# RainbowZL0/swin-unet-image-fusion

Measured on AMD Instinct MI355X. Metric: fused image-pairs/sec at 256x256, win=8, higher is better.
Workload: dtype bf16; 1 GPU; B=16/GPU 256x256 IR/visible pairs, win=8, 5-level Swin-UNet fusion forward (BASELINE configs[1]); global_batch=16, precision_mode=fast, residual_stream=fp32, hip_graph=True, steps_in_flight=3, kernel_schedule=throughput, collective=none, weights=random-init (numpy PCG64 recipe, seed 0)

## Files before the change

### swin_unet_image_fusion_amd/csrc/kernels_patchrr.hip

```cpp
#include "kernels_patchrr.h"

#include <algorithm>

#include "win_frag.h"

namespace swf {
namespace {

using namespace wf;

struct PrrArgs {
    const float* in[2]; float* out[2]; const float* skip[2]; const char* packed[2];
    int B, H, W, Cin;
    int mh, mw, Hm, Wm;
    int Ho, Wo;
    int K, N, Cout, M;
};

template <int KS, int NT>
struct PRR {
    static constexpr int NFRAG = NT * KS * 2;
    static constexpr int NV = NT * 16;
    static constexpr size_t p_vec = size_t(NFRAG) * 1024;
    static constexpr size_t p_total = p_vec + size_t(3) * 2 * NV * 4;
};

template <int KS, int NT, int DEC, int CIN1, int TPW>
__global__ __launch_bounds__(256) void patch_rr_kernel(PrrArgs a) {
    using P = PRR<KS, NT>;
    constexpr int NV = P::NV;
    __shared__ float lvec[3 * 2 * NV];
    const int s = blockIdx.y, tid = threadIdx.x, lane = tid & 63, wave = tid >> 6;
    const int r = lane & 31, hf = lane >> 5;
    fill_vectors<3 * NV / 4, 256>(lvec, a.packed[s] + P::p_vec, a.packed[s] + P::p_vec + (3 * NV / 4) * 16, tid);
    const __amdgpu_buffer_rsrc_t wrs = __builtin_amdgcn_make_buffer_rsrc(const_cast<char*>(a.packed[s]), 0, (int)P::p_total, 0x00020000);
    const unsigned loff = (unsigned)lane * 16u;
    auto WA = [&](int nt, int ks, int hl) {
        return __builtin_bit_cast(u32x4, __builtin_amdgcn_raw_buffer_load_b128(wrs, loff, ((nt * KS + ks) * 2 + hl) * 1024, 0));
    };
    __syncthreads();
    const float* vbias = lvec + hf * NV;
    const float* vgam = lvec + 2 * NV + hf * NV;
    const float* vbet = lvec + 4 * NV + hf * NV;
    const float* in = a.in[s];
    const int K = a.K, N = a.N, Cin = a.Cin;
    const float invN = 1.0f / (float)N;
    const f32x16 zero16 = {0.f, 0.f, 0.f, 0.f, 0.f, 0.f, 0.f, 0.f, 0.f, 0.f, 0.f, 0.f, 0.f, 0.f, 0.f, 0.f};

    const int ngroup = (a.M + 32 * TPW - 1) / (32 * TPW);
    for (int grp = blockIdx.x * 4 + wave; grp < ngroup; grp += gridDim.x * 4) {
        int tok[TPW], base[TPW][4];
        bool live[TPW];
#pragma unroll
        for (int u = 0; u < TPW; ++u) {
            const int t = (grp * TPW + u) * 32 + r;
            live[u] = t < a.M;
            const int tc = live[u] ? t : a.M - 1;
            tok[u] = tc;
            if constexpr (DEC) {
                const int mx = tc % a.Wm, t2 = tc / a.Wm, my = t2 % a.Hm, b = t2 / a.Hm;
                base[u][0] = ((b * a.H + my) * a.W + mx) * Cin;
                base[u][1] = base[u][2] = base[u][3] = 0;
            } else {
                const int ox = tc % a.Wo, t2 = tc / a.Wo, oy = t2 % a.Ho, b = t2 / a.Ho;
                const int my = reflect_br(oy, a.Hm), mx = reflect_br(ox, a.Wm);
                const int iy0 = reflect_br(2 * my, a.H), iy1 = reflect_br(2 * my + 1, a.H);
                const int ix0 = reflect_br(2 * mx, a.W), ix1 = reflect_br(2 * mx + 1, a.W);
                base[u][0] = ((b * a.H + iy0) * a.W + ix0) * Cin;
                base[u][1] = ((b * a.H + iy0) * a.W + ix1) * Cin;
                base[u][2] = ((b * a.H + iy1) * a.W + ix0) * Cin;
                base[u][3] = ((b * a.H + iy1) * a.W + ix1) * Cin;
            }
        }
        f32x16 acc[TPW][NT];
#pragma unroll
        for (int u = 0; u < TPW; ++u)
#pragma unroll
            for (int nt = 0; nt < NT; ++nt) acc[u][nt] = zero16;
        float xin[TPW][KS][8];
        {
            int pqk = 0, ck = 8 * hf;
            if constexpr (!DEC && !CIN1) {
                while (ck >= Cin) { ck -= Cin; ++pqk; }
            }
#pragma unroll
            for (int ks = 0; ks < KS; ++ks) {
#pragma unroll
                for (int u = 0; u < TPW; ++u) {
#pragma unroll
                    for (int j = 0; j < 8; ++j) xin[u][ks][j] = 0.f;
                    if constexpr (CIN1) {
                        if (hf == 0) {
                            xin[u][ks][0] = in[base[u][0]]; xin[u][ks][1] = in[base[u][1]];
                            xin[u][ks][2] = in[base[u][2]]; xin[u][ks][3] = in[base[u][3]];
                        }
                    } else {
                        const int k0 = 16 * ks + 8 * hf;
                        if (k0 < K) {
                            int off;
                            if constexpr (DEC) off = base[u][0] + k0;
                            else off = (pqk == 0 ? base[u][0] : pqk == 1 ? base[u][1] : pqk == 2 ? base[u][2] : base[u][3]) + ck;
                            const float4 x0 = *reinterpret_cast<const float4*>(in + off), x1 = *reinterpret_cast<const float4*>(in + off + 4);
                            xin[u][ks][0] = x0.x; xin[u][ks][1] = x0.y; xin[u][ks][2] = x0.z; xin[u][ks][3] = x0.w;
                            xin[u][ks][4] = x1.x; xin[u][ks][5] = x1.y; xin[u][ks][6] = x1.z; xin[u][ks][7] = x1.w;
                        }
                    }
                }
                if constexpr (!DEC && !CIN1) {
                    ck += 16;
                    while (ck >= Cin) { ck -= Cin; ++pqk; }
                }
            }
        }
        constexpr bool DEC_VEC = DEC != 0;
        constexpr bool SKIP_EARLY = DEC_VEC && NT <= 3;
        int oidx[DEC_VEC ? TPW : 1][DEC_VEC ? NT : 1][4];
        float4 skv[DEC_VEC ? TPW : 1][DEC_VEC ? NT : 1][4];
        auto dec_offsets = [&](int u) {
            const int t = tok[u];
            const int mx = t % a.Wm, t2 = t / a.Wm, my = t2 % a.Hm, b = t2 / a.Hm;
            int pq = 0, c = 4 * hf;
            while (c >= a.Cout) { c -= a.Cout; ++pq; }
#pragma unroll
            for (int nt = 0; nt < NT; ++nt)
#pragma unroll
                for (int g = 0; g < 4; ++g) {
                    const int yy = my * 2 + (pq >> 1), xx = mx * 2 + (pq & 1);
                    const bool ok = live[u] && 32 * nt + 8 * g + 4 * hf < N && yy < a.Ho && xx < a.Wo;
                    oidx[u][nt][g] = ok ? ((b * a.Ho + yy) * a.Wo + xx) * a.Cout + c : -1;
                    c += 8;
                    while (c >= a.Cout) { c -= a.Cout; ++pq; }
                }
        };
        auto load_skips = [&](int u) {
#pragma unroll
            for (int nt = 0; nt < NT; ++nt)
#pragma unroll
                for (int g = 0; g < 4; ++g)
                    skv[u][nt][g] = (a.skip[s] && oidx[u][nt][g] >= 0) ? *reinterpret_cast<const float4*>(a.skip[s] + oidx[u][nt][g])
                                                                       : make_float4(0.f, 0.f, 0.f, 0.f);
        };
        if constexpr (DEC_VEC) {
            if (a.Cout > 1) {
#pragma unroll
                for (int u = 0; u < TPW; ++u) {
                    dec_offsets(u);
                    if constexpr (SKIP_EARLY) load_skips(u);
                }
            }
        }
        u32x4 wr[2][NT][2];
        SWF_WF_FENCE();
#pragma unroll
        for (int nt = 0; nt < NT; ++nt) { wr[0][nt][0] = WA(nt, 0, 0); wr[0][nt][1] = WA(nt, 0, 1); }
#pragma unroll
        for (int ks = 0; ks < KS; ++ks) {
            if (ks + 1 < KS) {
#pragma unroll
                for (int nt = 0; nt < NT; ++nt) { wr[(ks + 1) & 1][nt][0] = WA(nt, ks + 1, 0); wr[(ks + 1) & 1][nt][1] = WA(nt, ks + 1, 1); }
            }
            SWF_WF_FENCE();
            u32x4 bh[TPW], bl[TPW];
#pragma unroll
            for (int u = 0; u < TPW; ++u) split8(xin[u][ks], bh[u], bl[u]);
#pragma unroll
            for (int nt = 0; nt < NT; ++nt)
#pragma unroll
                for (int u = 0; u < TPW; ++u) acc[u][nt] = mma3(wr[ks & 1][nt][0], wr[ks & 1][nt][1], bh[u], bl[u], acc[u][nt]);
        }
#pragma unroll
        for (int u = 0; u < TPW; ++u) {
            float sum = 0.f;
#pragma unroll
            for (int nt = 0; nt < NT; ++nt)
#pragma unroll
                for (int i = 0; i < 16; ++i) {
                    acc[u][nt][i] += vbias[nt * 16 + i];
                    sum += acc[u][nt][i];
                }
            const float mean = sum_halves(sum) * invN;
            float q = 0.f;
#pragma unroll
            for (int nt = 0; nt < NT; ++nt)
#pragma unroll
                for (int i = 0; i < 16; ++i) {
                    const float d = acc[u][nt][i] - mean;
                    q += (32 * nt + rho(i, hf) < N) ? d * d : 0.f;
                }
            const float rstd = __builtin_amdgcn_rsqf(sum_halves(q) * invN + 1e-5f);
            const int t = tok[u];
            if constexpr (DEC_VEC) {
                if (a.Cout > 1) {
                    if constexpr (!SKIP_EARLY) load_skips(u);
                }
            }
#pragma unroll
            for (int nt = 0; nt < NT; ++nt)
#pragma unroll
                for (int g = 0; g < 4; ++g) {
                    const int n0 = 32 * nt + 8 * g + 4 * hf;
                    if (n0 < N) {
                        float y[4];
#pragma unroll
                        for (int j = 0; j < 4; ++j) {
                            const int i = 4 * g + j;
                            const float z = (acc[u][nt][i] - mean) * rstd * vgam[nt * 16 + i] + vbet[nt * 16 + i];
                            y[j] = z > 0.f ? z : __builtin_amdgcn_exp2f(z * kLog2e) - 1.0f;
                        }
                        if constexpr (!DEC) {
                            if (live[u]) *reinterpret_cast<float4*>(a.out[s] + (int64_t)t * N + n0) = make_float4(y[0], y[1], y[2], y[3]);
                        } else if (a.Cout == 1) {
                            if (live[u]) {
                                const int mx = t % a.Wm, t2 = t / a.Wm, my = t2 % a.Hm, b = t2 / a.Hm;
#pragma unroll
                                for (int j = 0; j < 4; ++j) {
                                    const int yy = my * 2 + (j >> 1), xx = mx * 2 + (j & 1);
                                    if (yy < a.Ho && xx < a.Wo) {
                                        const int64_t o = ((int64_t)b * a.Ho + yy) * a.Wo + xx;
                                        a.out[s][o] = a.skip[s] ? y[j] + a.skip[s][o] : y[j];
                                    }
                                }
                            }
                        } else {
                            const int o = oidx[u][nt][g];
                            if (o >= 0) {
                                const float4 k4 = skv[u][nt][g];
                                *reinterpret_cast<float4*>(a.out[s] + o) = make_float4(y[0] + k4.x, y[1] + k4.y, y[2] + k4.z, y[3] + k4.w);
                            }
                        }
                    }
                }
        }
    }
}

struct PrrPackArgs { const float* w; const float* bias; const float* gamma; const float* beta; char* dst; int K, N; };

template <int KS, int NT>
__global__ __launch_bounds__(256) void patch_rr_pack_kernel(PrrPackArgs a) {
    using P = PRR<KS, NT>;
    const int gtid = blockIdx.x * blockDim.x + threadIdx.x, gsz = gridDim.x * blockDim.x;
    for (int idx = gtid; idx < P::NFRAG * 512; idx += gsz) {
        const int f = idx >> 9, lane = (idx >> 3) & 63, e = idx & 7, r = lane & 31, hf = lane >> 5;
        const int hl = f & 1, ks = (f >> 1) % KS, nt = f / (2 * KS);
        const int n = 32 * nt + r, k = 16 * ks + 8 * hf + e;
        const float val = (n < a.N && k < a.K) ? a.w[(int64_t)n * a.K + k] : 0.f;
        const bf16 hi = (bf16)val;
        reinterpret_cast<bf16*>(a.dst)[idx] = hl ? (bf16)(val - (float)hi) : hi;
    }
    float* vec = reinterpret_cast<float*>(a.dst + P::p_vec);
    for (int i = gtid; i < 3 * 2 * P::NV; i += gsz) {
        const int which = i / (2 * P::NV), hf = (i / P::NV) & 1, j = i % P::NV, nt = j >> 4, reg = j & 15;
        const int n = 32 * nt + rho(reg, hf);
        const float* src = which == 0 ? a.bias : which == 1 ? a.gamma : a.beta;
        vec[i] = (n < a.N && src) ? src[n] : 0.f;
    }
}

bool shape_class(int decoder, int Cin, int Cout, int mh, int mw, int* ks, int* nt) {
    if (mh != 2 || mw != 2 || Cin <= 0 || Cout <= 0) return false;
    const int K = decoder ? Cin : 4 * Cin, N = decoder ? 4 * Cout : Cout;
    if (decoder) {
        if (Cin % 8 || !(Cout == 1 || Cout % 4 == 0)) return false;
    } else {
        if (!(Cin == 1 || Cin % 8 == 0) || Cout % 4) return false;
    }
    *ks = (K + 15) / 16;
    *nt = (N + 31) / 32;
    const int k = *ks, n = *nt;
    if (decoder) return (k == 2 && n == 1) || (k == 3 && n == 3) || (k == 6 && n == 6);
    return (k == 1 && n == 1 && Cin == 1) || (k == 6 && n == 2) || (k == 12 && n == 3);
}

template <int KS, int NT, int DEC, int CIN1, int TPW>
int launch_t(const PrrArgs& a, int nstream, hipStream_t stream) {
    const int ngroup = (a.M + 32 * TPW - 1) / (32 * TPW);
    const int gx = std::max(1, std::min((ngroup + 3) / 4, 8 * num_cus() / nstream));
    hipLaunchKernelGGL((patch_rr_kernel<KS, NT, DEC, CIN1, TPW>), dim3(gx, nstream), dim3(256), 0, stream, a);
    return check_launch("patch_rr");
}

}

bool patch_rr_supported(int decoder, int Cin, int Cout, int mh, int mw) {
    int ks, nt;
    return shape_class(decoder, Cin, Cout, mh, mw, &ks, &nt);
}

size_t patch_rr_packed_bytes(int decoder, int Cin, int Cout, int mh, int mw) {
    int ks, nt;
    if (!shape_class(decoder, Cin, Cout, mh, mw, &ks, &nt)) return 0;
    return align_up(size_t(nt) * ks * 2 * 1024 + size_t(3) * 2 * nt * 16 * 4, 256);
}

int pack_patch_rr(int decoder, int Cin, int Cout, int mh, int mw, const float* weight, const float* bias, const float* gamma,
                  const float* beta, void* dst, hipStream_t stream) {
    int ks, nt;
    if (!shape_class(decoder, Cin, Cout, mh, mw, &ks, &nt)) return fail(SWF_ERR_UNSUPPORTED, "pack_patch_rr: shape not covered");
    PrrPackArgs a{weight, bias, gamma, beta, static_cast<char*>(dst), decoder ? Cin : 4 * Cin, decoder ? 4 * Cout : Cout};
#define SWF_PRR_PACK(KS_, NT_) if (ks == KS_ && nt == NT_) { hipLaunchKernelGGL((patch_rr_pack_kernel<KS_, NT_>), dim3(32), dim3(256), 0, stream, a); return check_launch("pack_patch_rr"); }
    SWF_PRR_PACK(1, 1) SWF_PRR_PACK(2, 1) SWF_PRR_PACK(3, 3) SWF_PRR_PACK(6, 2) SWF_PRR_PACK(6, 6) SWF_PRR_PACK(12, 3)
#undef SWF_PRR_PACK
    return fail(SWF_ERR_UNSUPPORTED, "pack_patch_rr: shape class");
}

int launch_patch_rr(const PatchFusedDesc& d, const void* const* packed, int nstream, hipStream_t stream) {
    int ks, nt;
    if (!shape_class(d.decoder, d.Cin, d.Cout, d.mh, d.mw, &ks, &nt)) return fail(SWF_ERR_UNSUPPORTED, "patch_rr: shape not covered");
    if (d.M <= 0 || d.M > INT32_MAX - 64) return fail(SWF_ERR_UNSUPPORTED, "patch_rr: token count");
    const int64_t in_elems = (int64_t)d.B * d.H * d.W * d.Cin;
    const int64_t out_elems = d.decoder ? (int64_t)d.B * d.Ho * d.Wo * d.Cout : d.M * (int64_t)d.N;
    if (in_elems >= (int64_t(1) << 31) || out_elems >= (int64_t(1) << 31)) return fail(SWF_ERR_UNSUPPORTED, "patch_rr: tensor too large");
    PrrArgs a{};
    uintptr_t bits = 0;
    for (int s = 0; s < nstream; ++s) {
        if (!packed || !packed[s]) return fail(SWF_ERR_NULL, "patch_rr: packed image missing");
        a.in[s] = d.in[s]; a.out[s] = d.out[s]; a.skip[s] = d.skip[s]; a.packed[s] = static_cast<const char*>(packed[s]);
        bits |= reinterpret_cast<uintptr_t>(d.in[s]) | reinterpret_cast<uintptr_t>(d.out[s]) | reinterpret_cast<uintptr_t>(d.skip[s]) |
                reinterpret_cast<uintptr_t>(packed[s]);
    }
    if (bits % 16) return fail(SWF_ERR_UNSUPPORTED, "patch_rr: tensors must be 16-byte aligned");
    a.B = d.B; a.H = d.H; a.W = d.W; a.Cin = d.Cin; a.mh = d.mh; a.mw = d.mw; a.Hm = d.Hm; a.Wm = d.Wm; a.Ho = d.Ho; a.Wo = d.Wo;
    a.K = d.K; a.N = d.N; a.Cout = d.Cout; a.M = (int)d.M;
    if (!d.decoder) {
        if (ks == 1 && nt == 1 && d.Cin == 1) return launch_t<1, 1, 0, 1, 2>(a, nstream, stream);
        if (ks == 6 && nt == 2) return launch_t<6, 2, 0, 0, 2>(a, nstream, stream);
        if (ks == 12 && nt == 3) return launch_t<12, 3, 0, 0, 1>(a, nstream, stream);
    } else {
        if (ks == 2 && nt == 1) return launch_t<2, 1, 1, 0, 2>(a, nstream, stream);
        if (ks == 3 && nt == 3) return launch_t<3, 3, 1, 0, 1>(a, nstream, stream);
        if (ks == 6 && nt == 6) return launch_t<6, 6, 1, 0, 1>(a, nstream, stream);
    }
    return fail(SWF_ERR_UNSUPPORTED, "patch_rr: no instantiation for k-steps %d, tiles %d (decoder %d)", ks, nt, d.decoder);
}

}
```

Before: 8971 pairs/s.

## Add software-pipelined patch-merge kernel with LDS-staged weights and input prefetch

Adds a pipelined variant of the fused patch-merge/expand kernel. It stages the packed weight and vector image into LDS once per block, then prefetches the next token group's inputs (and decoder skip values) while the current group's MMAs and LayerNorm/ELU epilogue run. By default it is used for two encoder shapes, the Cin=1 stem and the ks12/nt3 merge, each with its own blocks-per-CU grid setting. An env var can turn it off or route every shape through it. The cost is higher register pressure from the double-buffered inputs and dynamic LDS use, which can lower occupancy.

```diff
diff --git a/swin_unet_image_fusion_amd/csrc/kernels_patchrr.hip b/swin_unet_image_fusion_amd/csrc/kernels_patchrr.hip
--- a/swin_unet_image_fusion_amd/csrc/kernels_patchrr.hip
+++ b/swin_unet_image_fusion_amd/csrc/kernels_patchrr.hip
@@ -234,6 +234,270 @@
     }
 }
 
+template <int KS, int NT, int DEC, int CIN1, int TPW, int PF>
+__global__ __launch_bounds__(256) void patch_rr_pipe_kernel(PrrArgs a) {
+    using P = PRR<KS, NT>;
+    constexpr int NV = P::NV;
+    constexpr int TOTAL16 = (int)(P::p_total / 16), PER = (TOTAL16 + 255) / 256;
+    extern __shared__ __attribute__((aligned(16))) char prr_smem[];
+    const int s = blockIdx.y, tid = threadIdx.x, lane = tid & 63, wave = tid >> 6;
+    const int r = lane & 31, hf = lane >> 5;
+    const u32x4* lw = reinterpret_cast<const u32x4*>(prr_smem) + lane;
+    const float* lvec = reinterpret_cast<const float*>(prr_smem + P::p_vec);
+    const float* vbias = lvec + hf * NV;
+    const float* vgam = lvec + 2 * NV + hf * NV;
+    const float* vbet = lvec + 4 * NV + hf * NV;
+    const float* in = a.in[s];
+    const int K = a.K, N = a.N, Cin = a.Cin;
+    const float invN = 1.0f / (float)N;
+    const f32x16 zero16 = {0.f, 0.f, 0.f, 0.f, 0.f, 0.f, 0.f, 0.f, 0.f, 0.f, 0.f, 0.f, 0.f, 0.f, 0.f, 0.f};
+    constexpr bool DEC_VEC = DEC != 0;
+    const bool pair_in = CIN1 && !(a.W & 1) && 2 * a.Wm <= a.W;
+    const bool pair_out = DEC && a.Cout == 1 && !(a.Wo & 1);
+
+    int tok[TPW];
+    bool live[TPW];
+    float xin[TPW][KS][8];
+    int oidx[DEC_VEC ? TPW : 1][DEC_VEC ? NT : 1][4];
+    float4 skv[DEC_VEC ? TPW : 1][DEC_VEC ? NT : 1][4];
+
+    auto request = [&](int grp) {
+#pragma unroll
+        for (int u = 0; u < TPW; ++u) {
+            const int t = (grp * TPW + u) * 32 + r;
+            live[u] = t < a.M;
+            const int tc = live[u] ? t : a.M - 1;
+            tok[u] = tc;
+            int base[4];
+            if constexpr (DEC) {
+                const int mx = tc % a.Wm, t2 = tc / a.Wm, my = t2 % a.Hm, b = t2 / a.Hm;
+                base[0] = ((b * a.H + my) * a.W + mx) * Cin;
+                base[1] = base[2] = base[3] = 0;
+            } else {
+                const int ox = tc % a.Wo, t2 = tc / a.Wo, oy = t2 % a.Ho, b = t2 / a.Ho;
+                const int my = reflect_br(oy, a.Hm), mx = reflect_br(ox, a.Wm);
+                const int iy0 = reflect_br(2 * my, a.H), iy1 = reflect_br(2 * my + 1, a.H);
+                const int ix0 = reflect_br(2 * mx, a.W), ix1 = reflect_br(2 * mx + 1, a.W);
+                base[0] = ((b * a.H + iy0) * a.W + ix0) * Cin;
+                base[1] = ((b * a.H + iy0) * a.W + ix1) * Cin;
+                base[2] = ((b * a.H + iy1) * a.W + ix0) * Cin;
+                base[3] = ((b * a.H + iy1) * a.W + ix1) * Cin;
+            }
+            int pqk = 0, ck = 8 * hf;
+            if constexpr (!DEC && !CIN1) {
+                while (ck >= Cin) { ck -= Cin; ++pqk; }
+            }
+#pragma unroll
+            for (int ks = 0; ks < KS; ++ks) {
+#pragma unroll
+                for (int j = 0; j < 8; ++j) xin[u][ks][j] = 0.f;
+                if constexpr (CIN1) {
+                    if (hf == 0) {
+                        if (pair_in) {
+                            const float2 p0 = *reinterpret_cast<const float2*>(in + base[0]), p1 = *reinterpret_cast<const float2*>(in + base[2]);
+                            xin[u][ks][0] = p0.x; xin[u][ks][1] = p0.y; xin[u][ks][2] = p1.x; xin[u][ks][3] = p1.y;
+                        } else {
+                            xin[u][ks][0] = in[base[0]]; xin[u][ks][1] = in[base[1]];
+                            xin[u][ks][2] = in[base[2]]; xin[u][ks][3] = in[base[3]];
+                        }
+                    }
+                } else {
+                    const int k0 = 16 * ks + 8 * hf;
+                    if (k0 < K) {
+                        int off;
+                        if constexpr (DEC) off = base[0] + k0;
+                        else off = (pqk == 0 ? base[0] : pqk == 1 ? base[1] : pqk == 2 ? base[2] : base[3]) + ck;
+                        const float4 x0 = *reinterpret_cast<const float4*>(in + off), x1 = *reinterpret_cast<const float4*>(in + off + 4);
+                        xin[u][ks][0] = x0.x; xin[u][ks][1] = x0.y; xin[u][ks][2] = x0.z; xin[u][ks][3] = x0.w;
+                        xin[u][ks][4] = x1.x; xin[u][ks][5] = x1.y; xin[u][ks][6] = x1.z; xin[u][ks][7] = x1.w;
+                    }
+                    if constexpr (!DEC) {
+                        ck += 16;
+                        while (ck >= Cin) { ck -= Cin; ++pqk; }
+                    }
+                }
+            }
+            if constexpr (DEC_VEC) {
+                if (a.Cout > 1) {
+                    const int mx = tc % a.Wm, t2 = tc / a.Wm, my = t2 % a.Hm, b = t2 / a.Hm;
+                    int pq = 0, c = 4 * hf;
+                    while (c >= a.Cout) { c -= a.Cout; ++pq; }
+#pragma unroll
+                    for (int nt = 0; nt < NT; ++nt)
+#pragma unroll
+                        for (int g = 0; g < 4; ++g) {
+                            const int yy = my * 2 + (pq >> 1), xx = mx * 2 + (pq & 1);
+                            const bool ok = live[u] && 32 * nt + 8 * g + 4 * hf < N && yy < a.Ho && xx < a.Wo;
+                            oidx[u][nt][g] = ok ? ((b * a.Ho + yy) * a.Wo + xx) * a.Cout + c : -1;
+                            c += 8;
+                            while (c >= a.Cout) { c -= a.Cout; ++pq; }
+                        }
+#pragma unroll
+                    for (int nt = 0; nt < NT; ++nt)
+#pragma unroll
+                        for (int g = 0; g < 4; ++g)
+                            skv[u][nt][g] = (a.skip[s] && oidx[u][nt][g] >= 0) ? *reinterpret_cast<const float4*>(a.skip[s] + oidx[u][nt][g])
+                                                                               : make_float4(0.f, 0.f, 0.f, 0.f);
+                }
+            }
+        }
+    };
+
+    const int ngroup = (a.M + 32 * TPW - 1) / (32 * TPW), gstride = gridDim.x * 4;
+    int grp = blockIdx.x * 4 + wave;
+    {
+        f32x4 tmp[PER];
+#pragma unroll
+        for (int k = 0; k < PER; ++k) {
+            const int idx = tid + 256 * k;
+            if (idx < TOTAL16) tmp[k] = reinterpret_cast<const f32x4*>(a.packed[s])[idx];
+        }
+        SWF_WF_FENCE();
+        if (grp < ngroup) request(grp);
+        SWF_WF_FENCE();
+#pragma unroll
+        for (int k = 0; k < PER; ++k) {
+            const int idx = tid + 256 * k;
+            if (idx < TOTAL16) reinterpret_cast<f32x4*>(prr_smem)[idx] = tmp[k];
+        }
+    }
+    __syncthreads();
+    auto WL = [&](int q, int hl) { return lw[(q * 2 + hl) * 64]; };
+
+    for (; grp < ngroup; grp += gstride) {
+        int ctok[TPW];
+        bool clive[TPW];
+        int coidx[DEC_VEC ? TPW : 1][DEC_VEC ? NT : 1][4];
+        float4 cskv[DEC_VEC ? TPW : 1][DEC_VEC ? NT : 1][4];
+        u32x4 bh[TPW][KS], bl[TPW][KS];
+#pragma unroll
+        for (int u = 0; u < TPW; ++u) {
+            ctok[u] = tok[u];
+            clive[u] = live[u];
+            if constexpr (PF) {
+#pragma unroll
+                for (int ks = 0; ks < KS; ++ks) split8(xin[u][ks], bh[u][ks], bl[u][ks]);
+            }
+            if constexpr (DEC_VEC) {
+#pragma unroll
+                for (int nt = 0; nt < NT; ++nt)
+#pragma unroll
+                    for (int g = 0; g < 4; ++g) { coidx[u][nt][g] = oidx[u][nt][g]; cskv[u][nt][g] = skv[u][nt][g]; }
+            }
+        }
+        if constexpr (PF) {
+            SWF_WF_FENCE();
+            if (grp + gstride < ngroup) request(grp + gstride);
+            SWF_WF_FENCE();
+        }
+        f32x16 acc[TPW][NT];
+#pragma unroll
+        for (int u = 0; u < TPW; ++u)
+#pragma unroll
+            for (int nt = 0; nt < NT; ++nt) acc[u][nt] = zero16;
+        constexpr int NQ = KS * NT;
+        constexpr bool FENCED = NQ > 2;
+        u32x4 wr[3][2];
+        if constexpr (FENCED) SWF_WF_FENCE();
+        wr[0][0] = WL(0, 0); wr[0][1] = WL(0, 1);
+        if (NQ > 1) { wr[1][0] = WL((1 % NT) * KS + 1 / NT, 0); wr[1][1] = WL((1 % NT) * KS + 1 / NT, 1); }
+#pragma unroll
+        for (int q = 0; q < NQ; ++q) {
+            if (q + 2 < NQ) {
+                const int f = ((q + 2) % NT) * KS + (q + 2) / NT;
+                wr[(q + 2) % 3][0] = WL(f, 0); wr[(q + 2) % 3][1] = WL(f, 1);
+            }
+            if constexpr (FENCED) SWF_WF_FENCE();
+            const int nt = q % NT, ks = q / NT;
+            if constexpr (!PF) {
+                if (nt == 0) {
+#pragma unroll
+                    for (int u = 0; u < TPW; ++u) split8(xin[u][ks], bh[u][ks], bl[u][ks]);
+                }
+            }
+#pragma unroll
+            for (int u = 0; u < TPW; ++u) acc[u][nt] = mma3(wr[q % 3][0], wr[q % 3][1], bh[u][ks], bl[u][ks], acc[u][nt]);
+        }
+#pragma unroll
+        for (int u = 0; u < TPW; ++u) {
+            float sum = 0.f;
+#pragma unroll
+            for (int nt = 0; nt < NT; ++nt)
+#pragma unroll
+                for (int i = 0; i < 16; ++i) {
+                    acc[u][nt][i] += vbias[nt * 16 + i];
+                    sum += acc[u][nt][i];
+                }
+            const float mean = sum_halves(sum) * invN;
+            float q = 0.f;
+#pragma unroll
+            for (int nt = 0; nt < NT; ++nt)
+#pragma unroll
+                for (int i = 0; i < 16; ++i) {
+                    const float d = acc[u][nt][i] - mean;
+                    q += (32 * nt + rho(i, hf) < N) ? d * d : 0.f;
+                }
+            const float rstd = __builtin_amdgcn_rsqf(sum_halves(q) * invN + 1e-5f);
+            const int t = ctok[u];
+#pragma unroll
+            for (int nt = 0; nt < NT; ++nt)
+#pragma unroll
+                for (int g = 0; g < 4; ++g) {
+                    const int n0 = 32 * nt + 8 * g + 4 * hf;
+                    if (n0 < N) {
+                        float y[4];
+#pragma unroll
+                        for (int j = 0; j < 4; ++j) {
+                            const int i = 4 * g + j;
+                            const float z = (acc[u][nt][i] - mean) * rstd * vgam[nt * 16 + i] + vbet[nt * 16 + i];
+                            y[j] = z > 0.f ? z : __builtin_amdgcn_exp2f(z * kLog2e) - 1.0f;
+                        }
+                        if constexpr (!DEC) {
+                            if (clive[u]) *reinterpret_cast<float4*>(a.out[s] + (int64_t)t * N + n0) = make_float4(y[0], y[1], y[2], y[3]);
+                        } else if (a.Cout == 1) {
+                            if (clive[u]) {
+                                const int mx = t % a.Wm, t2 = t / a.Wm, my = t2 % a.Hm, b = t2 / a.Hm;
+                                if (pair_out) {
+#pragma unroll
+                                    for (int j = 0; j < 4; j += 2) {
+                                        const int yy = my * 2 + (j >> 1), xx = mx * 2;
+                                        if (yy < a.Ho && xx < a.Wo) {
+                                            const int64_t o = ((int64_t)b * a.Ho + yy) * a.Wo + xx;
+                                            float2 v = make_float2(y[j], y[j + 1]);
+                                            if (a.skip[s]) {
+                                                const float2 k2 = *reinterpret_cast<const float2*>(a.skip[s] + o);
+                                                v.x = y[j] + k2.x; v.y = y[j + 1] + k2.y;
+                                            }
+                                            *reinterpret_cast<float2*>(a.out[s] + o) = v;
+                                        }
+                                    }
+                                } else {
+#pragma unroll
+                                    for (int j = 0; j < 4; ++j) {
+                                        const int yy = my * 2 + (j >> 1), xx = mx * 2 + (j & 1);
+                                        if (yy < a.Ho && xx < a.Wo) {
+                                            const int64_t o = ((int64_t)b * a.Ho + yy) * a.Wo + xx;
+                                            a.out[s][o] = a.skip[s] ? y[j] + a.skip[s][o] : y[j];
+                                        }
+                                    }
+                                }
+                            }
+                        } else {
+                            const int o = coidx[u][nt][g];
+                            if (o >= 0) {
+                                const float4 k4 = cskv[u][nt][g];
+                                *reinterpret_cast<float4*>(a.out[s] + o) = make_float4(y[0] + k4.x, y[1] + k4.y, y[2] + k4.z, y[3] + k4.w);
+                            }
+                        }
+                    }
+                }
+        }
+        if constexpr (!PF) {
+            if (grp + gstride < ngroup) request(grp + gstride);
+        }
+    }
+}
+
 struct PrrPackArgs { const float* w; const float* bias; const float* gamma; const float* beta; char* dst; int K, N; };
 
 template <int KS, int NT>
@@ -278,6 +542,16 @@
     const int gx = std::max(1, std::min((ngroup + 3) / 4, 8 * num_cus() / nstream));
     hipLaunchKernelGGL((patch_rr_kernel<KS, NT, DEC, CIN1, TPW>), dim3(gx, nstream), dim3(256), 0, stream, a);
     return check_launch("patch_rr");
+}
+
+template <int KS, int NT, int DEC, int CIN1, int TPW, int PF>
+int launch_pipe_t(const PrrArgs& a, int nstream, hipStream_t stream, int bpc) {
+    const int ngroup = (a.M + 32 * TPW - 1) / (32 * TPW);
+    const int gx = std::max(1, std::min((ngroup + 3) / 4, bpc * num_cus() / nstream));
+    constexpr int lds = (int)PRR<KS, NT>::p_total;
+    if (lds > 65536) SWF_TRY((raise_lds_limit<&patch_rr_pipe_kernel<KS, NT, DEC, CIN1, TPW, PF>>(lds, "patch_rr_pipe")));
+    hipLaunchKernelGGL((patch_rr_pipe_kernel<KS, NT, DEC, CIN1, TPW, PF>), dim3(gx, nstream), dim3(256), lds, stream, a);
+    return check_launch("patch_rr_pipe");
 }
 
 }
@@ -322,14 +596,18 @@
     if (bits % 16) return fail(SWF_ERR_UNSUPPORTED, "patch_rr: tensors must be 16-byte aligned");
     a.B = d.B; a.H = d.H; a.W = d.W; a.Cin = d.Cin; a.mh = d.mh; a.mw = d.mw; a.Hm = d.Hm; a.Wm = d.Wm; a.Ho = d.Ho; a.Wo = d.Wo;
     a.K = d.K; a.N = d.N; a.Cout = d.Cout; a.M = (int)d.M;
+    static const int pipe = [] { const char* e = debug_env("SWF_PATCH_RR_PIPE"); return e ? std::atoi(e) : 1; }();
+    const bool all = pipe == 2, none = pipe == 0;
     if (!d.decoder) {
-        if (ks == 1 && nt == 1 && d.Cin == 1) return launch_t<1, 1, 0, 1, 2>(a, nstream, stream);
-        if (ks == 6 && nt == 2) return launch_t<6, 2, 0, 0, 2>(a, nstream, stream);
-        if (ks == 12 && nt == 3) return launch_t<12, 3, 0, 0, 1>(a, nstream, stream);
+        if (ks == 1 && nt == 1 && d.Cin == 1)
+            return none ? launch_t<1, 1, 0, 1, 2>(a, nstream, stream) : launch_pipe_t<1, 1, 0, 1, 2, 1>(a, nstream, stream, 4);
+        if (ks == 6 && nt == 2) return all ? launch_pipe_t<6, 2, 0, 0, 1, 1>(a, nstream, stream, 2) : launch_t<6, 2, 0, 0, 2>(a, nstream, stream);
+        if (ks == 12 && nt == 3)
+            return none ? launch_t<12, 3, 0, 0, 1>(a, nstream, stream) : launch_pipe_t<12, 3, 0, 0, 1, 0>(a, nstream, stream, 8);
     } else {
-        if (ks == 2 && nt == 1) return launch_t<2, 1, 1, 0, 2>(a, nstream, stream);
-        if (ks == 3 && nt == 3) return launch_t<3, 3, 1, 0, 1>(a, nstream, stream);
-        if (ks == 6 && nt == 6) return launch_t<6, 6, 1, 0, 1>(a, nstream, stream);
+        if (ks == 2 && nt == 1) return all ? launch_pipe_t<2, 1, 1, 0, 2, 1>(a, nstream, stream, 2) : launch_t<2, 1, 1, 0, 2>(a, nstream, stream);
+        if (ks == 3 && nt == 3) return all ? launch_pipe_t<3, 3, 1, 0, 1, 1>(a, nstream, stream, 1) : launch_t<3, 3, 1, 0, 1>(a, nstream, stream);
+        if (ks == 6 && nt == 6) return all ? launch_pipe_t<6, 6, 1, 0, 1, 0>(a, nstream, stream, 8) : launch_t<6, 6, 1, 0, 1>(a, nstream, stream);
     }
     return fail(SWF_ERR_UNSUPPORTED, "patch_rr: no instantiation for k-steps %d, tiles %d (decoder %d)", ks, nt, d.decoder);
 }
```

After: 8977 pairs/s, median of 6. Within noise of the previous version (+0.1%).
